# jyegerlehner/tensorflow-wavenet

Hardware: AMD Instinct MI355X
Metric: audio samples/sec (train, default wavenet_params.json) (higher is better)
Workload: dtype f32

## Files before the change

include/wavenet_hip.h:

```cpp
#ifndef WAVENET_HIP_H_
#define WAVENET_HIP_H_

#include <stdint.h>

#ifdef __cplusplus
extern "C" {
#endif

#define WN_OK 0
#define WN_ERR_BAD_SHAPE (-1)
#define WN_ERR_UNSUPPORTED (-2)
#define WN_ERR_MISALIGNED (-3)
#define WN_ERR_LAUNCH (-4)
#define WN_ERR_NULL (-5)

int wn_version(void);
const char* wn_error_string(int code);

int wn_mu_law_thresholds_host(int Q, float* thr_out);
int wn_mu_law_decode_table_host(int Q, float* lut_out);
int wn_mu_law_encode(const float* audio, int32_t* codes, long n,
                     const float* thr_dev, int Q, void* stream);
int wn_mu_law_decode(const int32_t* codes, float* audio, long n,
                     const float* lut_dev, int Q, void* stream);
// ... 82 lines not shown
                      int bias_clip_stride, const int* dilations, unsigned* flags,
                      unsigned* ctl, float* poison, int L, int B, int T, int save_sg,
                      int variant, const float* skip_img, const float* skip_bsum,
                      float* h1, void* stream);
int wn_stack_fwd_lc(float* X, float* Z, float* SG, const float* wimg,
                    const float* bias, long bias_layer_stride,
                    int bias_clip_stride, const int* dilations, unsigned* flags,
                    unsigned* ctl, float* poison, int L, int B, int T, int save_sg,
                    int variant, const float* lc_add, long lc_row_stride,
                    void* stream);
int wn_stack_bwd_slabs(int B, int T, int variant);
int wn_stack_fwd_waves(int B, int T, int variant);
int wn_stack_bwd_waves(int B, int T, int variant, int* tiles_per_wave);
int wn_stack_bwd(const float* X, const float* Z, const float* SG,
                 const float* dZ, float* DX, long dx_layer_stride, float* Q,
                 const float* wimg, float* slabs,
                 long slab_layer_stride, float* tilesum, const int* dilations,
                 unsigned* flags, unsigned* ctl, float* poison, int L, int B,
                 int T, int variant, void* stream);
int wn_stack_bwd_lc(const float* X, const float* Z, const float* SG,
                    const float* dZ, float* DX, long dx_layer_stride, float* Q,
                    const float* wimg, float* slabs,
                    long slab_layer_stride, float* tilesum, const int* dilations,
                    unsigned* flags, unsigned* ctl, float* poison, int L, int B,
                    int T, int variant, float* lc_da, long lc_row_stride,
                    void* stream);

int wn_gemm_nn(const float* A, long lda, int a_planes, long a_plane_stride,
               const float* W, int ldw, const float* bias, const float* mask,
               long ld_mask, const float* addend, long ld_add, float* C,
               long ldc, int c_planes, long c_plane_stride, float* Cpre,
               long M, int N, int K, int relu, void* stream);

long wn_gemm_split_w_bytes(int K, int N);
int wn_gemm_nn_split(const float* A, long lda, int a_planes,
                     long a_plane_stride, const float* W, int ldw,
                     const float* bias, const float* mask, long ld_mask,
                     const float* addend, long ld_add, float* C, long ldc,
                     int c_planes, long c_plane_stride, float* Cpre, long M,
                     int N, int K, int relu, void* w_scratch, int nprod,
                     void* stream);
long wn_gemm_tn_slab_floats(int Mw, int Nw);
int wn_gemm_tn_tail_rows(int Mw, int Nw);
int wn_gemm_tn_splits(long rows, int Mw, int Nw, int kind);
int wn_gemm_tn_split(const float* A, long lda, int a_planes,
                     long a_plane_stride, const float* G, long ldg,
                     float* slabs, int splits, long rows, int Mw, int Nw,
                     int want_colsum, int nprod, void* stream);
int wn_gemm_tn(const float* A, long lda, int a_planes, long a_plane_stride,
               const int32_t* codes, int shift, int T, const float* G,
               long ldg, float* slabs, int splits, long rows, int Mw, int Nw,
               int want_colsum, void* stream);
int wn_reduce_slabs(const float* slabs, int num_slabs, long slab_stride,
                    int batch, long in_batch_stride, long offset, long n,
                    float* dst, long out_batch_stride, int replicate,
                    long rep_stride, void* stream);
int wn_reduce_slabs_mt(const float* slabs, int num_slabs, long slab_stride,
                       long n_main, float* dst_main, long n_tail, float* dst_tail,
                       int replicate, long rep_stride, int tail_rows, void* stream);
int wn_reduce_pair_slabs(const float* slabs, int num_slabs, int CB, int K,
                         int has_dense, int use_bias, float* layer_grad, int C,
                         long off_bias, int tap0, int Ktot, void* stream);
int wn_transpose(const float* in, int rows, int cols, long in_ld, float* out,
                 long out_ld, void* stream);

int wn_xent_partials(long rows);
// ... 35 lines not shown
                     const float* l2_mask, const double* partials, int nparts,
                     float clip_norm, float* ema, float ema_decay,
                     float* norm_out, void* stream);
int wn_rmsprop_clip(float* p, const float* g, float* ms, float* mom, long n,
                    float lr, float decay, float momentum, float eps,
                    float grad_scale, float l2, const float* l2_mask,
                    const double* partials, int nparts, float clip_norm,
                    float* ema, float ema_decay, float* norm_out,
                    void* stream);
int wn_l2_partials_count(void);
int wn_l2_partials(const float* p, long n, const float* mask, float* partials,
                   void* stream);

int wn_gc_bias(const float* layer0, long layer_stride, long off_bias,
               long off_gc, int G, const float* emb, int card,
               const int32_t* ids, float* out, int L, int B, int ch,
               void* stream);
int wn_colsum_clip_chunks(int T);
int wn_colsum_clip(const float* plane0, const float* plane1, int B, int T,
                   float* part, float* out, void* stream);
int wn_gc_grad(const float* layer0, long layer_stride, long off_gc, int G,
               const float* emb, int card, const int32_t* ids,
               const float* dsum, int L, int B, float* glayer0, float* gemb,
               float* scratch , int ch, void* stream);

int wn_causal_conv(const float* x, const float* w, float* y, int B, int T,
                   int Cin, int Cout, int K, int dilation, void* stream);
int wn_time_to_batch(const float* in, float* out, int B, int T, int C,
                     int dilation, void* stream);
int wn_batch_to_time(const float* in, float* out, int B_out, int U, int C,
                     int dilation, void* stream);

int wn_diag_mfma_peak(float* out, int blocks, int iters, void* stream);

int wn_axpy(float* y, const float* x, float a, const float* mask, long n,
            void* stream);
int wn_fill(float* p, long n, float value, void* stream);
int wn_sum_rows(const float* in, int rows, int n, float* out, void* stream);

long wn_fastgen_state_floats(const int32_t* dilations_host, int L);
int wn_fastgen_init(float* state, long state_floats, int32_t* cursors, int L,
                    void* stream);
int wn_fastgen_run(const float* params_causal, const float* layer0,
                   long layer_stride, const float* skip_w,
                   const float* skip_bsum, const float* post1_w,
                   const float* post1_b, const float* post2_w,
                   const float* post2_b, const float* gc_bias_fg,
                   const int32_t* dilations_dev, int L, int S, int Q,
                   float* state, int32_t* cursors, int32_t* samples_io,
                   int n_given, int n_steps, float temperature, uint64_t seed,
                   float* proba_out, int proba_every, int use_biases,
                   int push, void* stream);

long wn_fastgen_wide_coop_bytes(int L, int C, int S, int Q);
int wn_fastgen_run_wide(const float* params_causal, const float* layer0,
                        long layer_stride, const float* skip_w,
                        const float* skip_bsum, const float* post1_w,
                        const float* post1_b, const float* post2_w,
                        const float* post2_b, const float* gc_bias_fg,
                        const int32_t* dilations_dev, int L, int C, int S, int Q,
                        float* state, int32_t* cursors, int32_t* samples_io,
                        int n_given, int n_steps, float temperature,
                        uint64_t seed, float* proba_out, int proba_every,
                        int use_biases, int push, void* coop, void* stream);

int wn_fastgen_step(const float* params_causal, const float* layer0,
// ... 228 lines not shown
```

tensorflow-wavenet_amd/csrc/wn_gemm.hip:

```cpp
#include "wn_common.h"
#include <cstdlib>
#include <cstddef>
#include <cstring>

struct GemmNN {
  const float* A;
  long lda;
  long a_plane_stride;
  int a_planes;
  const float* W;
  int ldw;
  const float* bias;
  const float* mask;
  long ld_mask;
  const float* addend;
  long ld_add;
  float* C;
  long ldc;
  long c_plane_stride;
  int c_planes;
  float* Cpre;
  long M;
  int N, K;
  int relu;
  int tiles_n;
  int nwg;
  int tiles_m;
  int tile_rows;
};

typedef const __attribute__((address_space(1))) void* gptr_t;
typedef __attribute__((address_space(3))) void* lptr_t;

#define NN_TM 128
#define NN_TN 128
#define NN_KC 32
#ifndef NN3_PF
#define NN3_PF 2
#endif

__device__ __forceinline__ int xcd_remap(int bid, int nwg) {
  const int q = nwg >> 3, r = nwg & 7, xcd = bid & 7, idx = bid >> 3;
  const int base = xcd < r ? xcd * (q + 1) : r * (q + 1) + (xcd - r) * q;
  return base + idx;
}

#define EP_LD 68
#ifndef EP_ST_AUX
#define EP_ST_AUX 2
#endif
#ifndef EP_LD_AUX
#define EP_LD_AUX 2
#endif
typedef unsigned ep_u32x4 __attribute__((ext_vector_type(4)));
__device__ __forceinline__ __amdgpu_buffer_rsrc_t ep_rsrc(const float* base) {
  return __builtin_amdgcn_make_buffer_rsrc((void*)base, 0, 0x7fffffff, 0x00020000);
}
__device__ __forceinline__ void gemm_epilogue(const GemmNN& g, f32x16 (&acc)[2][2],
                                              float* lds, long m0, int n0,
                                              int wm, int wn, int wave, int lane,
                                              long m_end = -1) {
  if (m_end < 0) m_end = g.M;
  const int j = lane & 31, h = lane >> 5;
  float* tile = lds + wave * (32 * EP_LD);
  const int rr = lane >> 4, cc = (lane & 15) * 4;
  const int nw = n0 + wn * 64;
  const bool ncol = nw + cc < g.N;
  f32x4 bias4 = {0.f, 0.f, 0.f, 0.f};
  if (g.bias && ncol) bias4 = *reinterpret_cast<const f32x4*>(g.bias + nw + cc);
  const int vC = g.c_planes ? (int)(((long)(cc >> 5) * g.c_plane_stride + rr * 32 + (cc & 31)) * 4)
                            : (int)((rr * g.ldc + cc) * 4);
  const int sC = g.c_planes ? 4 * 32 * 4 : (int)(4 * g.ldc * 4);
  const int vP = (int)((rr * g.ldc + cc) * 4);
  const int sP = (int)(4 * g.ldc * 4);
  const int vM = (int)((rr * g.ld_mask + cc) * 4), sM = (int)(4 * g.ld_mask * 4);
  const bool addp = g.addend && g.c_planes && g.ld_add == 0;
  const int vA = addp ? vC : (int)((rr * g.ld_add + cc) * 4);
  const int sA = addp ? sC : (int)(4 * g.ld_add * 4);
#pragma unroll
  for (int fm = 0; fm < 2; ++fm) {
    __builtin_amdgcn_wave_barrier();
#pragma unroll
    for (int fn = 0; fn < 2; ++fn)
#pragma unroll
      for (int q = 0; q < 4; ++q) {
        f32x4 v = {acc[fn][fm][4 * q], acc[fn][fm][4 * q + 1],
                   acc[fn][fm][4 * q + 2], acc[fn][fm][4 * q + 3]};
        *reinterpret_cast<f32x4*>(tile + j * EP_LD + fn * 32 + 8 * q + 4 * h) = v;
      }
    __builtin_amdgcn_wave_barrier();
    const long mbase = m0 + wm * 64 + fm * 32;
    const long left = m_end - mbase;
    const int nrows = left > 32 ? 32 : (left < 0 ? 0 : (int)left);
    const __amdgpu_buffer_rsrc_t rC = ep_rsrc(
        g.c_planes ? g.C + (long)(nw >> 5) * g.c_plane_stride + mbase * 32
                   : g.C + mbase * g.ldc + nw);
    const __amdgpu_buffer_rsrc_t rP = ep_rsrc(g.Cpre ? g.Cpre + mbase * g.ldc + nw : g.C);
    const __amdgpu_buffer_rsrc_t rM = ep_rsrc(g.mask ? g.mask + mbase * g.ld_mask + nw : g.C);
    const __amdgpu_buffer_rsrc_t rA = ep_rsrc(
        !g.addend ? g.C
        : addp ? g.addend + (long)(nw >> 5) * g.c_plane_stride + mbase * 32
               : g.addend + mbase * g.ld_add + nw);
#pragma unroll
    for (int bt = 0; bt < 2; ++bt) {
      f32x4 v[4], mk[4], ad[4];
#pragma unroll
      for (int q = 0; q < 4; ++q) {
        const int it = bt * 4 + q, row = it * 4 + rr;
        const bool ok = ncol && row < nrows;
        v[q] = *reinterpret_cast<const f32x4*>(tile + row * EP_LD + cc);
        if (g.mask && ok)
          mk[q] = __builtin_bit_cast(f32x4, __builtin_amdgcn_raw_buffer_load_b128(rM, vM, it * sM, EP_LD_AUX));
        if (g.addend && ok)
          ad[q] = __builtin_bit_cast(f32x4, __builtin_amdgcn_raw_buffer_load_b128(rA, vA, it * sA, EP_LD_AUX));
      }
#pragma unroll
      for (int q = 0; q < 4; ++q) {
        const int it = bt * 4 + q, row = it * 4 + rr;
        if (!(ncol && row < nrows)) continue;
        f32x4 x = v[q] + bias4;
        if (g.Cpre)
          __builtin_amdgcn_raw_buffer_store_b128(__builtin_bit_cast(ep_u32x4, x), rP, vP, it * sP, EP_ST_AUX);
        if (g.relu) {
#pragma unroll
// ... 181 lines not shown
    f32x16 fa[2];
#pragma unroll
    for (int fm = 0; fm < 2; ++fm) {
      const int row = wm * 64 + fm * 32 + j;
#pragma unroll
      for (int q = 0; q < 4; ++q) {
        const int sw = (2 * q + h) ^ ((j >> 1) & 7);
        const f32x4 v =
            *reinterpret_cast<const f32x4*>(&As[buf][row * NN_KC + sw * 4]);
        fa[fm][4 * q + 0] = v[0];
        fa[fm][4 * q + 1] = v[1];
        fa[fm][4 * q + 2] = v[2];
        fa[fm][4 * q + 3] = v[3];
      }
    }
    const float* bl = &Bs[buf][4 * h * NN_TN + wn * 64 + j];
#pragma unroll
    for (int r = 0; r < 16; ++r) {
      const int ko = (8 * (r >> 2) + (r & 3)) * NN_TN;
      const float w0 = bl[ko], w1 = bl[ko + 32];
      acc[0][0] = __builtin_amdgcn_mfma_f32_32x32x2f32(w0, fa[0][r], acc[0][0], 0, 0, 0);
      acc[0][1] = __builtin_amdgcn_mfma_f32_32x32x2f32(w0, fa[1][r], acc[0][1], 0, 0, 0);
      acc[1][0] = __builtin_amdgcn_mfma_f32_32x32x2f32(w1, fa[0][r], acc[1][0], 0, 0, 0);
      acc[1][1] = __builtin_amdgcn_mfma_f32_32x32x2f32(w1, fa[1][r], acc[1][1], 0, 0, 0);
    }
    if (kc + 1 < nk) sstore(buf ^ 1);
    __syncthreads();
  }

  gemm_epilogue(g, acc, smem, m0, n0, wm, wn, wave, lane);
}

#define N3_KC 16
#define N3_STAGE (NN_TM * N3_KC + N3_KC * NN_TN)

typedef __bf16 bf16x8 __attribute__((ext_vector_type(8)));
typedef unsigned int u32x4 __attribute__((ext_vector_type(4)));

struct Split3 {
  bf16x8 p[3];
};

__device__ __forceinline__ Split3 split3(const float (&v)[8]) {
  unsigned int hi[8], mi[8], lo[8];
#pragma unroll
  for (int e = 0; e < 8; ++e) {
    const unsigned int u = __float_as_uint(v[e]) & 0xffff0000u;
    const float r = v[e] - __uint_as_float(u);
    const unsigned int m = __float_as_uint(r) & 0xffff0000u;
    const float r2 = r - __uint_as_float(m);
    hi[e] = u;
    mi[e] = m;
    lo[e] = __float_as_uint(r2);
  }
  Split3 s;
  u32x4 ph, pm, pl;
#pragma unroll
  for (int w = 0; w < 4; ++w) {
    ph[w] = __builtin_amdgcn_perm(hi[2 * w + 1], hi[2 * w], 0x07060302u);
    pm[w] = __builtin_amdgcn_perm(mi[2 * w + 1], mi[2 * w], 0x07060302u);
    pl[w] = __builtin_amdgcn_perm(lo[2 * w + 1], lo[2 * w], 0x07060302u);
  }
  s.p[0] = __builtin_bit_cast(bf16x8, ph);
  s.p[1] = __builtin_bit_cast(bf16x8, pm);
  s.p[2] = __builtin_bit_cast(bf16x8, pl);
  return s;
}

template <int NPROD>
__device__ __forceinline__ void mma_split(f32x16& acc, const Split3& a, const Split3& b) {
#define WN_MM(i, k) \
  acc = __builtin_amdgcn_mfma_f32_32x32x16_bf16(a.p[i], b.p[k], acc, 0, 0, 0)
  if (NPROD >= 9) { WN_MM(2, 2); WN_MM(1, 2); WN_MM(2, 1); }
  if (NPROD >= 6) { WN_MM(1, 1); WN_MM(0, 2); WN_MM(2, 0); }
  WN_MM(0, 1);
  WN_MM(1, 0);
  WN_MM(0, 0);
#undef WN_MM
}

template <bool STAMPS>
__device__ __forceinline__ void nn3_tile(const GemmNN& g, float* smem, int tile_n, long m0,
                                         long m_end, unsigned long long* dbg) {
#define NSTAMP(i) if (STAMPS && threadIdx.x == 0) dbg[i] = __builtin_amdgcn_s_memtime()
  const int tid = threadIdx.x, lane = tid & 63;
  const int wave = __builtin_amdgcn_readfirstlane(tid >> 6);
  const int j = lane & 31, h = lane >> 5;
  const int wm = wave & 1, wn = wave >> 1;
  const int n0 = tile_n * NN_TN;
  const int nk = g.K / N3_KC;
  const bool live = n0 + wn * 64 < g.N;

  const int a_slot = lane & 3;
  const int a_chunk = a_slot ^ ((lane >> 4) & 3);
  long am0 = m0 + 16 * wave + (lane >> 2), am1 = am0 + 64;
  am0 = am0 < g.M ? am0 : g.M - 1;
  am1 = am1 < g.M ? am1 : g.M - 1;
  const long lda = g.a_planes ? 32 : g.lda;
  const int va0 = (int)((am0 * lda + a_chunk * 4) * 4);
  const int va1 = (int)((am1 * lda + a_chunk * 4) * 4);
  int wcol = n0 + (lane & 31) * 4;
  wcol = wcol < g.N ? wcol : 0;
  const int vw0 = (int)(((long)(2 * wave + (lane >> 5)) * g.ldw + wcol) * 4);
  const int vw1 = vw0 + (int)(8L * g.ldw * 4);
  auto stage = [&](int kc, float* base) {
    const __amdgpu_buffer_rsrc_t rsA = ep_rsrc(
        g.A + (g.a_planes ? (long)(kc >> 1) * g.a_plane_stride + (kc & 1) * 16 : (long)kc * N3_KC));
    const __amdgpu_buffer_rsrc_t rsW = ep_rsrc(g.W + (long)kc * N3_KC * g.ldw);
    __builtin_amdgcn_raw_ptr_buffer_load_lds(rsA, (lptr_t)(base + wave * 256), 16, va0, 0, 0, 0);
    __builtin_amdgcn_raw_ptr_buffer_load_lds(rsA, (lptr_t)(base + (wave + 4) * 256), 16, va1, 0, 0, 0);
    float* wb = base + NN_TM * N3_KC;
    __builtin_amdgcn_raw_ptr_buffer_load_lds(rsW, (lptr_t)(wb + wave * 256), 16, vw0, 0, 0, 0);
    __builtin_amdgcn_raw_ptr_buffer_load_lds(rsW, (lptr_t)(wb + (wave + 4) * 256), 16, vw1, 0, 0, 0);
  };

  f32x16 acc[2][2];
#pragma unroll
  for (int a = 0; a < 2; ++a)
#pragma unroll
    for (int b = 0; b < 2; ++b) acc[a][b] = frag_zero();

  stage(0, smem);
  if (!live) {
    for (int kc = 0; kc < nk; ++kc) {
      asm volatile("s_waitcnt vmcnt(0)\n\ts_barrier" ::: "memory");
      if (kc + 1 < nk) stage(kc + 1, smem + ((kc & 1) ^ 1) * N3_STAGE);
    }
  }
  for (int kc = 0; live && kc < nk; ++kc) {
    const int ST = kc & 1;
    asm volatile("s_waitcnt vmcnt(0)\n\ts_barrier" ::: "memory");
    if (STAMPS && kc == 0) { NSTAMP(1); }
    if (kc + 1 < nk) stage(kc + 1, smem + (ST ^ 1) * N3_STAGE);
    const float* As = smem + ST * N3_STAGE;
    const float* Bs = As + NN_TM * N3_KC;
    f32x4 fa[2][2];
#pragma unroll
    for (int fm = 0; fm < 2; ++fm) {
      const int row = wm * 64 + fm * 32 + j;
#pragma unroll
      for (int q = 0; q < 2; ++q)
        fa[fm][q] = *reinterpret_cast<const f32x4*>(
            As + row * N3_KC + (((2 * q + h) ^ ((row >> 2) & 3)) << 2));
    }
    const float* bl = Bs + 4 * h * NN_TN + wn * 64 + j;
    __builtin_amdgcn_s_setprio(1);
    constexpr int PF = NN3_PF;
    float wv[8][2];
#pragma unroll
    for (int r = 0; r < PF; ++r) {
      const int ko = (8 * (r >> 2) + (r & 3)) * NN_TN;
      wv[r][0] = bl[ko];
      wv[r][1] = bl[ko + 32];
    }
    __builtin_amdgcn_sched_barrier(0);
#pragma unroll
    for (int r = 0; r < 8; ++r) {
      if (r + PF < 8) {
        const int ko = (8 * ((r + PF) >> 2) + ((r + PF) & 3)) * NN_TN;
        wv[r + PF][0] = bl[ko];
        wv[r + PF][1] = bl[ko + 32];
      }
      __builtin_amdgcn_sched_barrier(0);
      const float w0 = wv[r][0], w1 = wv[r][1];
      const float x0 = fa[0][r >> 2][r & 3], x1 = fa[1][r >> 2][r & 3];
      acc[0][0] = __builtin_amdgcn_mfma_f32_32x32x2f32(w0, x0, acc[0][0], 0, 0, 0);
      acc[0][1] = __builtin_amdgcn_mfma_f32_32x32x2f32(w0, x1, acc[0][1], 0, 0, 0);
      acc[1][0] = __builtin_amdgcn_mfma_f32_32x32x2f32(w1, x0, acc[1][0], 0, 0, 0);
      acc[1][1] = __builtin_amdgcn_mfma_f32_32x32x2f32(w1, x1, acc[1][1], 0, 0, 0);
      __builtin_amdgcn_sched_barrier(0);
    }
    __builtin_amdgcn_s_setprio(0);
  }
  NSTAMP(2);
  asm volatile("s_waitcnt lgkmcnt(0)\n\ts_barrier" ::: "memory");
  NSTAMP(3);
  gemm_epilogue(g, acc, smem, m0, n0, wm, wn, wave, lane, m_end);
  NSTAMP(4);
#undef NSTAMP
}

constexpr int NN3_LDSF = 2 * N3_STAGE > 4 * 32 * EP_LD ? 2 * N3_STAGE : 4 * 32 * EP_LD;

__global__ __launch_bounds__(256, 4) void gemm_nn3_kernel(GemmNN g) {
  __shared__ __attribute__((aligned(1024))) float smem[NN3_LDSF];
  unsigned long long* dbg = nullptr;
#ifdef NN3_STAMPS
  dbg = reinterpret_cast<unsigned long long*>(g.Cpre) + (size_t)blockIdx.x * 8;
  g.Cpre = nullptr;
  if (threadIdx.x == 0) { dbg[0] = __builtin_amdgcn_s_memtime(); dbg[6] = __builtin_amdgcn_s_memrealtime(); }
#endif
  const int logical = xcd_remap(blockIdx.x, g.nwg);
  const int tile_n = logical % g.tiles_n;
  const long m0 = (long)(logical / g.tiles_n) * g.tile_rows;
  const long m_end = m0 + g.tile_rows < g.M ? m0 + g.tile_rows : g.M;
#ifdef NN3_STAMPS
  nn3_tile<true>(g, smem, tile_n, m0, m_end, dbg);
  if (threadIdx.x == 0) dbg[7] = __builtin_amdgcn_s_memrealtime();
#else
  nn3_tile<false>(g, smem, tile_n, m0, m_end, dbg);
#endif
}


#define S16_KC 32
#define S16_STAGE (NN_TM * S16_KC + 8 * 3 * 256)

__global__ void split_w_kernel(const float* __restrict__ W, int ldw, int K, int N,
                                 unsigned int* __restrict__ out, int nt16) {
  const int kc = blockIdx.y, nt = blockIdx.x, lane = threadIdx.x;
  const int n = nt * 16 + (lane & 15);
  float v[8];
#pragma unroll
  for (int e = 0; e < 8; ++e) {
    const int k = kc * S16_KC + 8 * (lane >> 4) + e;
    v[e] = (k < K && n < N) ? W[(long)k * ldw + n] : 0.f;
  }
  const Split3 s = split3(v);
  u32x4* dst = reinterpret_cast<u32x4*>(out) + ((long)(kc * nt16 + nt) * 3) * 64 + lane;
#pragma unroll
  for (int p = 0; p < 3; ++p) dst[p * 64] = __builtin_bit_cast(u32x4, s.p[p]);
}

template <int NPROD>
__device__ __forceinline__ void mma_split16(f32x4& acc, const Split3& a, const Split3& b) {
#define WN_MM(i, k) \
  acc = __builtin_amdgcn_mfma_f32_16x16x32_bf16(a.p[i], b.p[k], acc, 0, 0, 0)
  if (NPROD >= 9) { WN_MM(2, 2); WN_MM(1, 2); WN_MM(2, 1); }
  if (NPROD >= 6) { WN_MM(1, 1); WN_MM(0, 2); WN_MM(2, 0); }
  WN_MM(0, 1);
  WN_MM(1, 0);
  WN_MM(0, 0);
#undef WN_MM
// ... 955 lines not shown
static int gemm_nn_describe(GemmNN& g, const float* A, long lda, int a_planes,
               long a_plane_stride, const float* W, int ldw, const float* bias,
               const float* mask, long ld_mask, const float* addend, long ld_add,
               float* C, long ldc, int c_planes, long c_plane_stride, float* Cpre,
               long M, int N, int K, int relu) {
  if (!A || !W || !C) return WN_ERR_NULL;
  if (M <= 0 || N <= 0 || K <= 0) return WN_ERR_BAD_SHAPE;
  if ((N & 3) || (K & 3) || (ldw & 3)) return WN_ERR_UNSUPPORTED;
  if (a_planes) {
    if (K != a_planes * 32) return WN_ERR_BAD_SHAPE;
  } else if (lda & 3) {
    return WN_ERR_UNSUPPORTED;
  }
  if (c_planes) {
    if (N != c_planes * 32) return WN_ERR_BAD_SHAPE;
  } else if (ldc & 3) {
    return WN_ERR_UNSUPPORTED;
  }
  if ((mask && (ld_mask & 3)) || (addend && (ld_add & 3)))
    return WN_ERR_UNSUPPORTED;
  if (addend && ld_add == 0 && !c_planes) return WN_ERR_BAD_SHAPE;
  if (c_planes && c_plane_stride * 4 >= (1L << 31)) return WN_ERR_UNSUPPORTED;
  const void* ptrs[] = {A, W, bias, mask, addend, C, Cpre};
  for (const void* p : ptrs)
    if (p && !wn_aligned16(p)) return WN_ERR_MISALIGNED;
  g.A = A; g.lda = lda; g.a_plane_stride = a_plane_stride; g.a_planes = a_planes;
  g.W = W; g.ldw = ldw; g.bias = bias; g.mask = mask; g.ld_mask = ld_mask;
  g.addend = addend; g.ld_add = ld_add; g.C = C; g.ldc = ldc;
  g.c_plane_stride = c_plane_stride; g.c_planes = c_planes; g.Cpre = Cpre;
  g.M = M; g.N = N; g.K = K; g.relu = relu;
  long tiles_m = (M + NN_TM - 1) / NN_TM;
  g.tiles_n = (N + NN_TN - 1) / NN_TN;
  g.tile_rows = NN_TM;
  const long nwg = tiles_m * g.tiles_n;
  if (nwg > 0x7fffffffL) return WN_ERR_BAD_SHAPE;
  g.nwg = (int)nwg;
  g.tiles_m = (int)tiles_m;
  return WN_OK;
}

static bool gemm_nn3_ok(const GemmNN& g) {
  const long a_bytes = (g.a_planes ? g.M * 32 : g.M * g.lda) * 4;
  return (g.K % N3_KC) == 0 && a_bytes < (1L << 31) &&
         (long)N3_KC * g.ldw * 4 < (1L << 31);
}

static int gemm_nn_launch(const float* A, long lda, int a_planes, long a_plane_stride,
               const float* W, int ldw, const float* bias, const float* mask,
               long ld_mask, const float* addend, long ld_add, float* C,
               long ldc, int c_planes, long c_plane_stride, float* Cpre,
               long M, int N, int K, int relu, void* stream,
               void* wsplit = nullptr, int nprod = 0) {
  GemmNN g;
  const int rc = gemm_nn_describe(g, A, lda, a_planes, a_plane_stride, W, ldw, bias, mask,
                                  ld_mask, addend, ld_add, C, ldc, c_planes,
                                  c_plane_stride, Cpre, M, N, K, relu);
  if (rc != WN_OK) return rc;
  const long nwg = g.nwg;
  if (wsplit && (K % N3_KC) != 0) return WN_ERR_UNSUPPORTED;
  if (wsplit && !wn_aligned16(wsplit)) return WN_ERR_MISALIGNED;
  if (!wsplit && !gemm_nn3_ok(g))
    hipLaunchKernelGGL(gemm_nn_kernel<2>, dim3((unsigned)nwg), dim3(256), 0,
                       (hipStream_t)stream, g);
  else if (wsplit) {
    hipStream_t s = (hipStream_t)stream;
    dim3 gr((unsigned)nwg), bl(256);
    const unsigned int* wp = (const unsigned int*)wsplit;
    const int nt16 = (N + 15) / 16;
    hipLaunchKernelGGL(split_w_kernel, dim3(nt16, (K + S16_KC - 1) / S16_KC), dim3(64), 0, s,
                       W, ldw, K, N, (unsigned int*)wsplit, nt16);
    if (nprod == 3) hipLaunchKernelGGL(gemm_nn_split_kernel<3>, gr, bl, 0, s, g, wp, nt16);
    else if (nprod == 9) hipLaunchKernelGGL(gemm_nn_split_kernel<9>, gr, bl, 0, s, g, wp, nt16);
    else hipLaunchKernelGGL(gemm_nn_split_kernel<6>, gr, bl, 0, s, g, wp, nt16);
  } else
    hipLaunchKernelGGL(gemm_nn3_kernel, dim3((unsigned)nwg), dim3(256), 0,
                       (hipStream_t)stream, g);
  return wn_check_launch();
}

int wn_gemm_nn(const float* A, long lda, int a_planes, long a_plane_stride,
               const float* W, int ldw, const float* bias, const float* mask,
               long ld_mask, const float* addend, long ld_add, float* C,
               long ldc, int c_planes, long c_plane_stride, float* Cpre,
               long M, int N, int K, int relu, void* stream) {
  return gemm_nn_launch(A, lda, a_planes, a_plane_stride, W, ldw, bias, mask,
                        ld_mask, addend, ld_add, C, ldc, c_planes,
                        c_plane_stride, Cpre, M, N, K, relu, stream);
}

long wn_gemm_split_w_bytes(int K, int N) {
  if (K <= 0 || N <= 0) return 0;
  return (long)((K + 31) / 32) * ((N + 15) / 16) * 3 * 1024;
}

int wn_gemm_nn_split(const float* A, long lda, int a_planes, long a_plane_stride,
                     const float* W, int ldw, const float* bias, const float* mask,
                     long ld_mask, const float* addend, long ld_add, float* C,
                     long ldc, int c_planes, long c_plane_stride, float* Cpre,
                     long M, int N, int K, int relu, void* w_scratch, int nprod,
                     void* stream) {
  if (!w_scratch) return WN_ERR_NULL;
  if (nprod != 3 && nprod != 6 && nprod != 9) return WN_ERR_BAD_SHAPE;
  return gemm_nn_launch(A, lda, a_planes, a_plane_stride, W, ldw, bias, mask,
                        ld_mask, addend, ld_add, C, ldc, c_planes,
                        c_plane_stride, Cpre, M, N, K, relu, stream, w_scratch,
                        nprod);
}



static int tn_device_cus() { return wn_device_cus(); }

static bool tn_wg_tile(int Mw, int Nw, int* mf, int* nf);

int wn_gemm_tn_tail_rows(int Mw, int Nw) {
  int mf = 0, nf = 0;
  if (Mw <= 0 || Nw <= 0 || !tn_wg_tile(Mw, Nw, &mf, &nf)) return 1;
  return Mw / (mf * 32);
}

// ... 234 lines not shown
```

tensorflow-wavenet_amd/wavenet/_lib.py:

```python
import ctypes
import os

_HERE = os.path.dirname(os.path.abspath(__file__))
LIB_PATH = os.environ.get('WN_LIB_PATH') or os.path.join(
    os.path.dirname(_HERE), 'libwavenet_hip.so')

c_int, c_long, c_float = ctypes.c_int, ctypes.c_long, ctypes.c_float
c_void_p, c_u64 = ctypes.c_void_p, ctypes.c_uint64
P = c_void_p

SIGNATURES = {
    'wn_version': (c_int, []),
    'wn_error_string': (ctypes.c_char_p, [c_int]),
    'wn_mu_law_thresholds_host': (c_int, [c_int, P]),
    'wn_mu_law_decode_table_host': (c_int, [c_int, P]),
    'wn_mu_law_encode': (c_int, [P, P, c_long, P, c_int, P]),
    'wn_mu_law_decode': (c_int, [P, P, c_long, P, c_int, P]),
    'wn_causal_gather': (c_int, [P, P, P, c_int, c_int, c_int, c_int, c_int,
                                 P]),
    'wn_scalar_causal_fwd': (c_int, [P, P, c_int, P, c_int, c_int, c_int, P]),
    'wn_scalar_causal_wgrad': (c_int, [P, P, P, c_int, c_int, c_int, c_int,
                                       P]),
    'wn_causal_wgrad_slabs': (c_int, [c_long]),
    'wn_causal_wgrad': (c_int, [P, P, P, c_int, c_int, c_int, c_int, P]),
# ... 17 lines not shown
    'wn_stack_fwd_waves': (c_int, [c_int, c_int, c_int]),
    'wn_stack_bwd_waves': (c_int, [c_int, c_int, c_int, P]),
    'wn_stack_bwd': (c_int, [P, P, P, P, P, c_long, P, P, P, c_long, P, P, P,
                             P, P, c_int, c_int, c_int, c_int, P]),
    'wn_stack_bwd_lc': (c_int, [P, P, P, P, P, c_long, P, P, P, c_long, P, P,
                                P, P, P, c_int, c_int, c_int, c_int, P, c_long,
                                P]),
    'wn_layer_wgrad_slab_floats': (c_int, []),
    'wn_dense_planes': (c_int, [P, c_long, P, P, P, c_long, P, c_long, c_long, c_int,
                                P]),
    'wn_dense_planes_gate': (c_int, [P, c_long, P, P, c_long, P, P, c_long, P, P,
                                     c_long, c_long, c_int, P]),
    'wn_layer_fwd_k': (c_int, [P, P, P, P, P, P, P, c_int, c_int, c_int, c_int,
                               c_int, c_int, c_int, P]),
    'wn_layer_bwd_k': (c_int, [P, P, P, P, P, P, P, P, P, P, P, c_int, c_int,
                               c_int, c_int, c_int, c_int, c_int, c_long, P]),
    'wn_layer_wgrad_k': (c_int, [P, P, P, P, P, P, c_int, c_int, c_int, c_int,
                                 c_int, c_int, c_int, c_int, c_long, P]),
    'wn_layer_fwd_blk': (c_int, [P, c_long, c_int, P, P, P, P, P, c_int, P, P,
                                 c_int, c_int, c_int, c_int, c_int, c_int,
                                 c_int, P, P, c_long, c_int, c_int, c_int,
                                 c_long, P]),
    'wn_layer_bwd_blk': (c_int, [P, P, c_long, c_int, P, P, P, P, c_int,
                                 c_long, c_int, c_int, c_int, c_int, c_int,
                                 c_int, c_int, c_long, P]),
    'wn_layer_bwd2_slabs': (c_int, [c_int, c_int]),
    'wn_layer_bwd2_wimg_floats': (c_int, []),
    'wn_layer_bwd2_pack': (c_int, [P, c_long, P, c_int, P]),
    'wn_layer_bwd2': (c_int, [P, P, P, P, P, P, P, P, P, P, c_int, c_int,
                              c_int, P]),
    'wn_gemm_nn': (c_int, [P, c_long, c_int, c_long, P, c_int, P, P, c_long,
                           P, c_long, P, c_long, c_int, c_long, P, c_long,
                           c_int, c_int, c_int, P]),
    'wn_gemm_split_w_bytes': (c_long, [c_int, c_int]),
    'wn_gemm_nn_split': (c_int, [P, c_long, c_int, c_long, P, c_int, P, P,
                                 c_long, P, c_long, P, c_long, c_int, c_long,
                                 P, c_long, c_int, c_int, c_int, P, c_int, P]),
    'wn_gemm_tn_tail_rows': (c_int, [c_int, c_int]),
    'wn_gemm_tn_slab_floats': (c_long, [c_int, c_int]),
    'wn_gemm_tn_splits': (c_int, [c_long, c_int, c_int, c_int]),
    'wn_gemm_tn_split': (c_int, [P, c_long, c_int, c_long, P, c_long, P, c_int,
                                 c_long, c_int, c_int, c_int, c_int, P]),
    'wn_gemm_tn': (c_int, [P, c_long, c_int, c_long, P, c_int, c_int, P,
                           c_long, P, c_int, c_long, c_int, c_int, c_int, P]),
    'wn_reduce_slabs': (c_int, [P, c_int, c_long, c_int, c_long, c_long,
                                c_long, P, c_long, c_int, c_long, P]),
    'wn_reduce_slabs_mt': (c_int, [P, c_int, c_long, c_long, P, c_long, P, c_int,
                                   c_long, c_int, P]),
    'wn_reduce_pair_slabs': (c_int, [P, c_int, c_int, c_int, c_int, c_int, P,
                                     c_int, c_long, c_int, c_int, P]),
    'wn_transpose': (c_int, [P, c_int, c_int, c_long, P, c_long, P]),
    'wn_xent_partials': (c_int, [c_long]),
    'wn_xent': (c_int, [P, c_long, P, P, P, c_int, c_int, c_int, c_int, P]),
    'wn_xent_masked': (c_int, [P, c_long, P, P, P, P, P, c_int, c_int, c_int,
                               c_int, P]),
    'wn_xent_score_scratch_floats': (c_long, [c_long]),
    'wn_xent_score': (c_int, [P, c_long, P, P, P, P, P, P, P, c_int, c_int,
                              c_int, P]),
    'wn_softmax64_row': (c_int, [P, c_int, P, P]),
    'wn_adam': (c_int, [P, P, P, P, c_long, c_float, c_float, c_float,
                        c_float, c_float, c_float, P, P]),
    'wn_momentum': (c_int, [P, P, P, c_long, c_float, c_float, c_float,
                            c_float, P, P]),
    'wn_rmsprop': (c_int, [P, P, P, P, c_long, c_float, c_float, c_float,
                           c_float, c_float, c_float, P, P]),
    'wn_grad_norm_partials_count': (c_int, []),
    'wn_grad_norm_partials': (c_int, [P, c_long, P, P]),
    'wn_adam_clip': (c_int, [P, P, P, P, c_long, c_float, c_float, c_float,
                             c_float, c_float, c_float, P, P, c_int, c_float,
                             P, c_float, P, P]),
    'wn_momentum_clip': (c_int, [P, P, P, c_long, c_float, c_float, c_float,
                                 c_float, P, P, c_int, c_float, P, c_float, P,
                                 P]),
    'wn_rmsprop_clip': (c_int, [P, P, P, P, c_long, c_float, c_float, c_float,
                                c_float, c_float, c_float, P, P, c_int,
                                c_float, P, c_float, P, P]),
    'wn_l2_partials_count': (c_int, []),
    'wn_l2_partials': (c_int, [P, c_long, P, P, P]),
    'wn_gc_bias': (c_int, [P, c_long, c_long, c_long, c_int, P, c_int, P, P,
                           c_int, c_int, c_int, P]),
    'wn_colsum_clip_chunks': (c_int, [c_int]),
    'wn_colsum_clip': (c_int, [P, P, c_int, c_int, P, P, P]),
    'wn_gc_grad': (c_int, [P, c_long, c_long, c_int, P, c_int, P, P, c_int,
                           c_int, P, P, P, c_int, P]),
    'wn_causal_conv': (c_int, [P, P, P, c_int, c_int, c_int, c_int, c_int,
                               c_int, P]),
    'wn_time_to_batch': (c_int, [P, P, c_int, c_int, c_int, c_int, P]),
    'wn_batch_to_time': (c_int, [P, P, c_int, c_int, c_int, c_int, P]),
    'wn_diag_mfma_peak': (c_int, [P, c_int, c_int, P]),
    'wn_axpy': (c_int, [P, P, c_float, P, c_long, P]),
    'wn_fill': (c_int, [P, c_long, c_float, P]),
    'wn_sum_rows': (c_int, [P, c_int, c_int, P, P]),
    'wn_fastgen_state_floats': (c_long, [P, c_int]),
    'wn_fastgen_init': (c_int, [P, c_long, P, c_int, P]),
    'wn_fastgen_run': (c_int, [P, P, c_long, P, P, P, P, P, P, P, P, c_int,
                               c_int, c_int, P, P, P, c_int, c_int, c_float,
                               c_u64, P, c_int, c_int, c_int, P]),
    'wn_fastgen_run_wide': (c_int, [P, P, c_long, P, P, P, P, P, P, P, P,
                                    c_int, c_int, c_int, c_int, P, P, P, c_int,
                                    c_int, c_float, c_u64, P, c_int, c_int,
                                    c_int, P, P]),
    'wn_fastgen_wide_coop_bytes': (c_long, [c_int, c_int, c_int, c_int]),
    'wn_fastgen_step': (c_int, [P, P, c_long, P, P, P, P, P, P, P, P, c_int,
                                c_int, c_int, P, P, P, P, P, c_int, P, P, P,
                                P, P, P, P]),
    'wn_fastgen_persist_workgroups': (c_int, [c_int, c_int, c_int]),
    'wn_fastgen_persist_role': (c_int, [c_int, c_int, c_int]),
    'wn_fastgen_persist_ll_words': (c_long, [c_int, c_int, c_int]),
    'wn_fastgen_persist': (c_int, [P, P, c_long, P, P, P, P, P, P, P, P, c_int,
                                   c_int, c_int, P, P, P, P, P, c_int, P, P, P,
                                   P, P, P, P, P, c_int, P]),
    'wn_fastgen_pre': (c_int, [P, c_long, P, P, c_int, P, P, P, P]),
    'wn_fastgen_finish': (c_int, [c_int, P, P, P, P, P, P]),
    'wn_fastgen_pack': (c_int, [P, c_long, P, c_int, P]),
    'wn_fastgen_batch_rows': (c_int, [c_int]),
    'wn_fastgen_batch_state_floats': (c_long, [P, c_int, c_int]),
    'wn_fastgen_batch_init': (c_int, [P, c_long, P, P, c_int, P]),
    'wn_fastgen_batch_pre': (c_int, [P, c_long, P, c_int, P, c_int, c_int, P,
                                     P, P, P]),
    'wn_fastgen_batch_step': (c_int, [P, P, c_long, P, P, P, P, P, P, P,
                                      c_int, P, c_int, c_int, c_int, c_int, P,
                                      P, P, P, P, P, P, c_int, P, P, P, P, P,
# ... 172 lines not shown
```

Measured before the change: 13.35 million.

## Plan mixed 128/64-row tiles in NN GEMM to balance wave quantization

Adds a host-side planner that picks how many 256-row groups use 128x128 tiles and switches the remainder (or everything, for small grids) to 64-row tiles so workgroups fill the CU slots more evenly across rounds. The nn3 tile routine is templated on tile shape and wave layout, handles a 64-column edge tile as a 256x64 tile, and drops the idle-wave path for dead columns. The goal is less tail idling in the last partial round of workgroups. The cost is extra index math in the kernel and smaller tiles with less operand reuse for the remainder. A diagnostic entry point that forces a plan is also added.

Result: no change. 13.33 million (-0.2%).

```diff
diff --git a/include/wavenet_hip.h b/include/wavenet_hip.h
--- a/include/wavenet_hip.h
+++ b/include/wavenet_hip.h
@@ -138,6 +138,8 @@
                long ldc, int c_planes, long c_plane_stride, float* Cpre,
                long M, int N, int K, int relu, void* stream);
 
+int wn_gemm_nn_plan(long M, int N, int K, int* tile_rows, long* rem_start);
+
 long wn_gemm_split_w_bytes(int K, int N);
 int wn_gemm_nn_split(const float* A, long lda, int a_planes,
                      long a_plane_stride, const float* W, int ldw,
@@ -239,6 +241,13 @@
                      int dilation, void* stream);
 
 int wn_diag_mfma_peak(float* out, int blocks, int iters, void* stream);
+int wn_diag_gemm_nn_planned(const float* A, long lda, int a_planes,
+                            long a_plane_stride, const float* W, int ldw,
+                            const float* bias, const float* mask, long ld_mask,
+                            const float* addend, long ld_add, float* C,
+                            long ldc, int c_planes, long c_plane_stride,
+                            float* Cpre, long M, int N, int K, int relu,
+                            long rem_start, void* stream);
 
 int wn_axpy(float* y, const float* x, float a, const float* mask, long n,
             void* stream);
diff --git a/tensorflow-wavenet_amd/csrc/wn_gemm.hip b/tensorflow-wavenet_amd/csrc/wn_gemm.hip
--- a/tensorflow-wavenet_amd/csrc/wn_gemm.hip
+++ b/tensorflow-wavenet_amd/csrc/wn_gemm.hip
@@ -27,6 +27,7 @@
   int nwg;
   int tiles_m;
   int tile_rows;
+  int head_groups;
 };
 
 typedef const __attribute__((address_space(1))) void* gptr_t;
@@ -35,6 +36,9 @@
 #define NN_TM 128
 #define NN_TN 128
 #define NN_KC 32
+#ifndef NN3_T64_WAVES
+#define NN3_T64_WAVES 4
+#endif
 #ifndef NN3_PF
 #define NN3_PF 2
 #endif
@@ -56,7 +60,8 @@
 __device__ __forceinline__ __amdgpu_buffer_rsrc_t ep_rsrc(const float* base) {
   return __builtin_amdgcn_make_buffer_rsrc((void*)base, 0, 0x7fffffff, 0x00020000);
 }
-__device__ __forceinline__ void gemm_epilogue(const GemmNN& g, f32x16 (&acc)[2][2],
+template <int FM = 2>
+__device__ __forceinline__ void gemm_epilogue(const GemmNN& g, f32x16 (&acc)[2][FM],
                                               float* lds, long m0, int n0,
                                               int wm, int wn, int wave, int lane,
                                               long m_end = -1) {
@@ -78,7 +83,7 @@
   const int vA = addp ? vC : (int)((rr * g.ld_add + cc) * 4);
   const int sA = addp ? sC : (int)(4 * g.ld_add * 4);
 #pragma unroll
-  for (int fm = 0; fm < 2; ++fm) {
+  for (int fm = 0; fm < FM; ++fm) {
     __builtin_amdgcn_wave_barrier();
 #pragma unroll
     for (int fn = 0; fn < 2; ++fn)
@@ -89,7 +94,7 @@
         *reinterpret_cast<f32x4*>(tile + j * EP_LD + fn * 32 + 8 * q + 4 * h) = v;
       }
     __builtin_amdgcn_wave_barrier();
-    const long mbase = m0 + wm * 64 + fm * 32;
+    const long mbase = m0 + wm * (32 * FM) + fm * 32;
     const long left = m_end - mbase;
     const int nrows = left > 32 ? 32 : (left < 0 ? 0 : (int)left);
     const __amdgpu_buffer_rsrc_t rC = ep_rsrc(
@@ -337,7 +342,10 @@
 }
 
 #define N3_KC 16
-#define N3_STAGE (NN_TM * N3_KC + N3_KC * NN_TN)
+#define NN_GROUP 256
+constexpr int NN3_LDSF = 2 * (NN_GROUP * N3_KC + N3_KC * 64);
+static_assert(NN3_LDSF >= 2 * (NN_TM * N3_KC + N3_KC * NN_TN) && NN3_LDSF >= 4 * 32 * EP_LD,
+              "LDS of gemm_nn3_kernel");
 
 typedef __bf16 bf16x8 __attribute__((ext_vector_type(8)));
 typedef unsigned int u32x4 __attribute__((ext_vector_type(4)));
@@ -384,77 +392,81 @@
 #undef WN_MM
 }
 
-template <bool STAMPS>
-__device__ __forceinline__ void nn3_tile(const GemmNN& g, float* smem, int tile_n, long m0,
+template <int TM, int TN, int WM, int FM, bool STAMPS, int NW = 4>
+__device__ __forceinline__ void nn3_tile(const GemmNN& g, float* smem, int n0, long m0,
                                          long m_end, unsigned long long* dbg) {
 #define NSTAMP(i) if (STAMPS && threadIdx.x == 0) dbg[i] = __builtin_amdgcn_s_memtime()
+  static_assert(TM == WM * FM * 32 && TN == (NW / WM) * 64, "wave layout");
+  constexpr int STAGE = TM * N3_KC + N3_KC * TN;
+  static_assert(2 * STAGE <= NN3_LDSF, "operand stages");
+  constexpr int PA = TM / 16 / NW;
+  constexpr int CW = TN / 4;
+  constexpr int KR = 64 / CW;
+  constexpr int PW = N3_KC / KR / NW;
   const int tid = threadIdx.x, lane = tid & 63;
   const int wave = __builtin_amdgcn_readfirstlane(tid >> 6);
   const int j = lane & 31, h = lane >> 5;
-  const int wm = wave & 1, wn = wave >> 1;
-  const int n0 = tile_n * NN_TN;
+  const int wm = wave % WM, wn = wave / WM;
   const int nk = g.K / N3_KC;
-  const bool live = n0 + wn * 64 < g.N;
+  if (NW < 4 && wave >= NW) return;
 
   const int a_slot = lane & 3;
   const int a_chunk = a_slot ^ ((lane >> 4) & 3);
-  long am0 = m0 + 16 * wave + (lane >> 2), am1 = am0 + 64;
-  am0 = am0 < g.M ? am0 : g.M - 1;
-  am1 = am1 < g.M ? am1 : g.M - 1;
   const long lda = g.a_planes ? 32 : g.lda;
-  const int va0 = (int)((am0 * lda + a_chunk * 4) * 4);
-  const int va1 = (int)((am1 * lda + a_chunk * 4) * 4);
-  int wcol = n0 + (lane & 31) * 4;
+  int va[PA];
+#pragma unroll
+  for (int i = 0; i < PA; ++i) {
+    long am = m0 + 16 * (wave + NW * i) + (lane >> 2);
+    am = am < g.M ? am : g.M - 1;
+    va[i] = (int)((am * lda + a_chunk * 4) * 4);
+  }
+  int wcol = n0 + (lane % CW) * 4;
   wcol = wcol < g.N ? wcol : 0;
-  const int vw0 = (int)(((long)(2 * wave + (lane >> 5)) * g.ldw + wcol) * 4);
-  const int vw1 = vw0 + (int)(8L * g.ldw * 4);
+  const int vw0 = (int)(((long)(KR * wave + lane / CW) * g.ldw + wcol) * 4);
+  const int vws = (int)((long)NW * KR * g.ldw * 4);
   auto stage = [&](int kc, float* base) {
     const __amdgpu_buffer_rsrc_t rsA = ep_rsrc(
         g.A + (g.a_planes ? (long)(kc >> 1) * g.a_plane_stride + (kc & 1) * 16 : (long)kc * N3_KC));
     const __amdgpu_buffer_rsrc_t rsW = ep_rsrc(g.W + (long)kc * N3_KC * g.ldw);
-    __builtin_amdgcn_raw_ptr_buffer_load_lds(rsA, (lptr_t)(base + wave * 256), 16, va0, 0, 0, 0);
-    __builtin_amdgcn_raw_ptr_buffer_load_lds(rsA, (lptr_t)(base + (wave + 4) * 256), 16, va1, 0, 0, 0);
-    float* wb = base + NN_TM * N3_KC;
-    __builtin_amdgcn_raw_ptr_buffer_load_lds(rsW, (lptr_t)(wb + wave * 256), 16, vw0, 0, 0, 0);
-    __builtin_amdgcn_raw_ptr_buffer_load_lds(rsW, (lptr_t)(wb + (wave + 4) * 256), 16, vw1, 0, 0, 0);
+#pragma unroll
+    for (int i = 0; i < PA; ++i)
+      __builtin_amdgcn_raw_ptr_buffer_load_lds(rsA, (lptr_t)(base + (wave + NW * i) * 256), 16, va[i], 0, 0, 0);
+    float* wb = base + TM * N3_KC;
+#pragma unroll
+    for (int i = 0; i < PW; ++i)
+      __builtin_amdgcn_raw_ptr_buffer_load_lds(rsW, (lptr_t)(wb + (wave + NW * i) * 256), 16, vw0 + i * vws, 0, 0, 0);
   };
 
-  f32x16 acc[2][2];
+  f32x16 acc[2][FM];
 #pragma unroll
   for (int a = 0; a < 2; ++a)
 #pragma unroll
-    for (int b = 0; b < 2; ++b) acc[a][b] = frag_zero();
+    for (int b = 0; b < FM; ++b) acc[a][b] = frag_zero();
 
   stage(0, smem);
-  if (!live) {
-    for (int kc = 0; kc < nk; ++kc) {
-      asm volatile("s_waitcnt vmcnt(0)\n\ts_barrier" ::: "memory");
-      if (kc + 1 < nk) stage(kc + 1, smem + ((kc & 1) ^ 1) * N3_STAGE);
-    }
-  }
-  for (int kc = 0; live && kc < nk; ++kc) {
+  for (int kc = 0; kc < nk; ++kc) {
     const int ST = kc & 1;
     asm volatile("s_waitcnt vmcnt(0)\n\ts_barrier" ::: "memory");
     if (STAMPS && kc == 0) { NSTAMP(1); }
-    if (kc + 1 < nk) stage(kc + 1, smem + (ST ^ 1) * N3_STAGE);
-    const float* As = smem + ST * N3_STAGE;
-    const float* Bs = As + NN_TM * N3_KC;
-    f32x4 fa[2][2];
-#pragma unroll
-    for (int fm = 0; fm < 2; ++fm) {
-      const int row = wm * 64 + fm * 32 + j;
+    if (kc + 1 < nk) stage(kc + 1, smem + (ST ^ 1) * STAGE);
+    const float* As = smem + ST * STAGE;
+    const float* Bs = As + TM * N3_KC;
+    f32x4 fa[FM][2];
+#pragma unroll
+    for (int fm = 0; fm < FM; ++fm) {
+      const int row = wm * (32 * FM) + fm * 32 + j;
 #pragma unroll
       for (int q = 0; q < 2; ++q)
         fa[fm][q] = *reinterpret_cast<const f32x4*>(
             As + row * N3_KC + (((2 * q + h) ^ ((row >> 2) & 3)) << 2));
     }
-    const float* bl = Bs + 4 * h * NN_TN + wn * 64 + j;
+    const float* bl = Bs + 4 * h * TN + wn * 64 + j;
     __builtin_amdgcn_s_setprio(1);
     constexpr int PF = NN3_PF;
     float wv[8][2];
 #pragma unroll
     for (int r = 0; r < PF; ++r) {
-      const int ko = (8 * (r >> 2) + (r & 3)) * NN_TN;
+      const int ko = (8 * (r >> 2) + (r & 3)) * TN;
       wv[r][0] = bl[ko];
       wv[r][1] = bl[ko + 32];
     }
@@ -462,17 +474,18 @@
 #pragma unroll
     for (int r = 0; r < 8; ++r) {
       if (r + PF < 8) {
-        const int ko = (8 * ((r + PF) >> 2) + ((r + PF) & 3)) * NN_TN;
+        const int ko = (8 * ((r + PF) >> 2) + ((r + PF) & 3)) * TN;
         wv[r + PF][0] = bl[ko];
         wv[r + PF][1] = bl[ko + 32];
       }
       __builtin_amdgcn_sched_barrier(0);
       const float w0 = wv[r][0], w1 = wv[r][1];
-      const float x0 = fa[0][r >> 2][r & 3], x1 = fa[1][r >> 2][r & 3];
-      acc[0][0] = __builtin_amdgcn_mfma_f32_32x32x2f32(w0, x0, acc[0][0], 0, 0, 0);
-      acc[0][1] = __builtin_amdgcn_mfma_f32_32x32x2f32(w0, x1, acc[0][1], 0, 0, 0);
-      acc[1][0] = __builtin_amdgcn_mfma_f32_32x32x2f32(w1, x0, acc[1][0], 0, 0, 0);
-      acc[1][1] = __builtin_amdgcn_mfma_f32_32x32x2f32(w1, x1, acc[1][1], 0, 0, 0);
+#pragma unroll
+      for (int fm = 0; fm < FM; ++fm)
+        acc[0][fm] = __builtin_amdgcn_mfma_f32_32x32x2f32(w0, fa[fm][r >> 2][r & 3], acc[0][fm], 0, 0, 0);
+#pragma unroll
+      for (int fm = 0; fm < FM; ++fm)
+        acc[1][fm] = __builtin_amdgcn_mfma_f32_32x32x2f32(w1, fa[fm][r >> 2][r & 3], acc[1][fm], 0, 0, 0);
       __builtin_amdgcn_sched_barrier(0);
     }
     __builtin_amdgcn_s_setprio(0);
@@ -480,12 +493,10 @@
   NSTAMP(2);
   asm volatile("s_waitcnt lgkmcnt(0)\n\ts_barrier" ::: "memory");
   NSTAMP(3);
-  gemm_epilogue(g, acc, smem, m0, n0, wm, wn, wave, lane, m_end);
+  gemm_epilogue<FM>(g, acc, smem, m0, n0, wm, wn, wave, lane, m_end);
   NSTAMP(4);
 #undef NSTAMP
 }
-
-constexpr int NN3_LDSF = 2 * N3_STAGE > 4 * 32 * EP_LD ? 2 * N3_STAGE : 4 * 32 * EP_LD;
 
 __global__ __launch_bounds__(256, 4) void gemm_nn3_kernel(GemmNN g) {
   __shared__ __attribute__((aligned(1024))) float smem[NN3_LDSF];
@@ -495,15 +506,37 @@
   g.Cpre = nullptr;
   if (threadIdx.x == 0) { dbg[0] = __builtin_amdgcn_s_memtime(); dbg[6] = __builtin_amdgcn_s_memrealtime(); }
 #endif
-  const int logical = xcd_remap(blockIdx.x, g.nwg);
-  const int tile_n = logical % g.tiles_n;
-  const long m0 = (long)(logical / g.tiles_n) * g.tile_rows;
-  const long m_end = m0 + g.tile_rows < g.M ? m0 + g.tile_rows : g.M;
 #ifdef NN3_STAMPS
-  nn3_tile<true>(g, smem, tile_n, m0, m_end, dbg);
+  constexpr bool ST = true;
+#else
+  constexpr bool ST = false;
+#endif
+  const int edge = (g.N % NN_TN) == 64, cols_n = g.tiles_n - edge;
+  const int head_wgs = g.head_groups * (NN_GROUP / 128 * cols_n + edge);
+  const bool head = (int)blockIdx.x < head_wgs;
+  const int rows = head ? 128 : 64;
+  const int per = NN_GROUP / rows * cols_n + edge;
+  const int logical = head ? xcd_remap(blockIdx.x, head_wgs)
+                           : xcd_remap(blockIdx.x - head_wgs, g.nwg - head_wgs);
+  const int grp = logical / per + (head ? 0 : g.head_groups), r = logical % per;
+  const long mg = (long)grp * NN_GROUP;
+  if (edge && r == per - 1) {
+    const long m_end = mg + NN_GROUP < g.M ? mg + NN_GROUP : g.M;
+    nn3_tile<NN_GROUP, 64, 4, 2, ST>(g, smem, cols_n * NN_TN, mg, m_end, dbg);
+  } else {
+    const long m0 = mg + (long)(r / cols_n) * rows;
+    if (m0 >= g.M) return;
+    const long m_end = m0 + rows < g.M ? m0 + rows : g.M;
+    const int n0 = (r % cols_n) * NN_TN;
+    if (head) nn3_tile<128, 128, 2, 2, ST>(g, smem, n0, m0, m_end, dbg);
+#if NN3_T64_WAVES == 2
+    else nn3_tile<64, 128, 1, 2, ST, 2>(g, smem, n0, m0, m_end, dbg);
+#else
+    else nn3_tile<64, 128, 2, 1, ST>(g, smem, n0, m0, m_end, dbg);
+#endif
+  }
+#ifdef NN3_STAMPS
   if (threadIdx.x == 0) dbg[7] = __builtin_amdgcn_s_memrealtime();
-#else
-  nn3_tile<false>(g, smem, tile_n, m0, m_end, dbg);
 #endif
 }
 
@@ -1525,6 +1558,7 @@
   long tiles_m = (M + NN_TM - 1) / NN_TM;
   g.tiles_n = (N + NN_TN - 1) / NN_TN;
   g.tile_rows = NN_TM;
+  g.head_groups = 0;
   const long nwg = tiles_m * g.tiles_n;
   if (nwg > 0x7fffffffL) return WN_ERR_BAD_SHAPE;
   g.nwg = (int)nwg;
@@ -1538,14 +1572,70 @@
          (long)N3_KC * g.ldw * 4 < (1L << 31);
 }
 
+#define NN3_FILL_64 0.5
+#define NN3_MIX_REM 0.6
+#define NN3_MIX_ROUNDS 4
+
+struct Nn3Plan {
+  int tile_rows;
+  long rem_start;
+};
+
+static long nn3_group_wgs(int N, int rows) {
+  const int edge = (N % NN_TN) == 64;
+  return (long)(NN_GROUP / rows) * (edge ? N / NN_TN : (N + NN_TN - 1) / NN_TN) + edge;
+}
+
+static Nn3Plan nn3_plan(long M, int N, int K, int cus) {
+  const long groups = (M + NN_GROUP - 1) / NN_GROUP;
+  Nn3Plan p = {NN_TM, groups * NN_GROUP};
+  if ((K % N3_KC) != 0) return p;
+  const long slots = 4L * cus;
+  const int edge = (N % NN_TN) == 64;
+  const long cols = edge ? N / NN_TN : (N + NN_TN - 1) / NN_TN;
+  const long wg128 = (M + NN_TM - 1) / NN_TM * cols + edge * groups;
+  if (wg128 <= (long)(NN3_FILL_64 * slots)) {
+    p.tile_rows = 64;
+    p.rem_start = 0;
+    return p;
+  }
+  const long full = wg128 / slots, rem = wg128 % slots;
+  if (full == 0 || rem == 0 || rem > (long)(NN3_MIX_REM * slots) || full > NN3_MIX_ROUNDS)
+    return p;
+  const long head = full * slots / nn3_group_wgs(N, NN_TM);
+  if (head < groups) p.rem_start = head * NN_GROUP;
+  return p;
+}
+
+static int nn3_plan_fill(GemmNN& g, const Nn3Plan& p) {
+  const long groups = (g.M + NN_GROUP - 1) / NN_GROUP;
+  long head = p.rem_start / NN_GROUP;
+  head = head < groups ? head : groups;
+  const long nwg = head * nn3_group_wgs(g.N, 128) + (groups - head) * nn3_group_wgs(g.N, 64);
+  if (nwg > 0x7fffffffL) return WN_ERR_BAD_SHAPE;
+  g.head_groups = (int)head;
+  g.nwg = (int)nwg;
+  return WN_OK;
+}
+
+int wn_gemm_nn_plan(long M, int N, int K, int* tile_rows, long* rem_start) {
+  if (!tile_rows || !rem_start) return WN_ERR_NULL;
+  if (M <= 0 || N <= 0 || K <= 0) return WN_ERR_BAD_SHAPE;
+  const Nn3Plan p = nn3_plan(M, N, K, wn_device_cus());
+  *tile_rows = p.tile_rows;
+  *rem_start = p.rem_start;
+  return WN_OK;
+}
+
 static int gemm_nn_launch(const float* A, long lda, int a_planes, long a_plane_stride,
                const float* W, int ldw, const float* bias, const float* mask,
                long ld_mask, const float* addend, long ld_add, float* C,
                long ldc, int c_planes, long c_plane_stride, float* Cpre,
                long M, int N, int K, int relu, void* stream,
-               void* wsplit = nullptr, int nprod = 0) {
+               void* wsplit = nullptr, int nprod = 0,
+               const Nn3Plan* forced = nullptr) {
   GemmNN g;
-  const int rc = gemm_nn_describe(g, A, lda, a_planes, a_plane_stride, W, ldw, bias, mask,
+  int rc = gemm_nn_describe(g, A, lda, a_planes, a_plane_stride, W, ldw, bias, mask,
                                   ld_mask, addend, ld_add, C, ldc, c_planes,
                                   c_plane_stride, Cpre, M, N, K, relu);
   if (rc != WN_OK) return rc;
@@ -1565,9 +1655,12 @@
     if (nprod == 3) hipLaunchKernelGGL(gemm_nn_split_kernel<3>, gr, bl, 0, s, g, wp, nt16);
     else if (nprod == 9) hipLaunchKernelGGL(gemm_nn_split_kernel<9>, gr, bl, 0, s, g, wp, nt16);
     else hipLaunchKernelGGL(gemm_nn_split_kernel<6>, gr, bl, 0, s, g, wp, nt16);
-  } else
-    hipLaunchKernelGGL(gemm_nn3_kernel, dim3((unsigned)nwg), dim3(256), 0,
+  } else {
+    rc = nn3_plan_fill(g, forced ? *forced : nn3_plan(M, N, K, wn_device_cus()));
+    if (rc != WN_OK) return rc;
+    hipLaunchKernelGGL(gemm_nn3_kernel, dim3((unsigned)g.nwg), dim3(256), 0,
                        (hipStream_t)stream, g);
+  }
   return wn_check_launch();
 }
 
@@ -1579,6 +1672,21 @@
   return gemm_nn_launch(A, lda, a_planes, a_plane_stride, W, ldw, bias, mask,
                         ld_mask, addend, ld_add, C, ldc, c_planes,
                         c_plane_stride, Cpre, M, N, K, relu, stream);
+}
+
+int wn_diag_gemm_nn_planned(const float* A, long lda, int a_planes, long a_plane_stride,
+               const float* W, int ldw, const float* bias, const float* mask,
+               long ld_mask, const float* addend, long ld_add, float* C,
+               long ldc, int c_planes, long c_plane_stride, float* Cpre,
+               long M, int N, int K, int relu, long rem_start, void* stream) {
+  if (rem_start % NN_GROUP) return WN_ERR_BAD_SHAPE;
+  const long a_bytes = (a_planes ? M * 32 : M * lda) * 4;
+  if (K <= 0 || (K % N3_KC) || a_bytes >= (1L << 31) || (long)N3_KC * ldw * 4 >= (1L << 31))
+    return WN_ERR_UNSUPPORTED;
+  const Nn3Plan p = {rem_start <= 0 ? 64 : NN_TM, rem_start <= 0 ? 0 : rem_start};
+  return gemm_nn_launch(A, lda, a_planes, a_plane_stride, W, ldw, bias, mask,
+                        ld_mask, addend, ld_add, C, ldc, c_planes,
+                        c_plane_stride, Cpre, M, N, K, relu, stream, nullptr, 0, &p);
 }
 
 long wn_gemm_split_w_bytes(int K, int N) {
diff --git a/tensorflow-wavenet_amd/wavenet/_lib.py b/tensorflow-wavenet_amd/wavenet/_lib.py
--- a/tensorflow-wavenet_amd/wavenet/_lib.py
+++ b/tensorflow-wavenet_amd/wavenet/_lib.py
@@ -73,6 +73,7 @@
     'wn_gemm_nn': (c_int, [P, c_long, c_int, c_long, P, c_int, P, P, c_long,
                            P, c_long, P, c_long, c_int, c_long, P, c_long,
                            c_int, c_int, c_int, P]),
+    'wn_gemm_nn_plan': (c_int, [c_long, c_int, c_int, P, P]),
     'wn_gemm_split_w_bytes': (c_long, [c_int, c_int]),
     'wn_gemm_nn_split': (c_int, [P, c_long, c_int, c_long, P, c_int, P, P,
                                  c_long, P, c_long, P, c_long, c_int, c_long,
@@ -129,6 +130,10 @@
     'wn_time_to_batch': (c_int, [P, P, c_int, c_int, c_int, c_int, P]),
     'wn_batch_to_time': (c_int, [P, P, c_int, c_int, c_int, c_int, P]),
     'wn_diag_mfma_peak': (c_int, [P, c_int, c_int, P]),
+    'wn_diag_gemm_nn_planned': (c_int, [P, c_long, c_int, c_long, P, c_int, P, P,
+                                        c_long, P, c_long, P, c_long, c_int,
+                                        c_long, P, c_long, c_int, c_int, c_int,
+                                        c_long, P]),
     'wn_axpy': (c_int, [P, P, c_float, P, c_long, P]),
     'wn_fill': (c_int, [P, c_long, c_float, P]),
     'wn_sum_rows': (c_int, [P, c_int, c_int, P, P]),
```
